# anovos/anovos

Measured on AMD Instinct MI355X. Metric: rows/sec (whole node) full analyzer+drift+transform, higher is better.
Workload: dtype fp32 data + fp64 accumulators; 1 GPU; model=anovos-full-pipeline, rows_per_gpu=125000000, n_cols=201, global_batch=125000000, parallelism=dp1

## Files before the change

anovos_amd/data_analyzer/association_evaluator.py:

```python

from __future__ import annotations

import math
import warnings

import numpy as np
import pandas as pd
import torch

from anovos_amd.core import dist
from anovos_amd.core.dtypes import NULL_CODE
from anovos_amd.data_analyzer.association_eval_varclus import VarClusHi
from anovos_amd.data_analyzer.stats_generator import uniqueCount_computation
from anovos_amd.data_transformer.transformers import (
    attribute_binning,
    cat_to_num_unsupervised,
    imputation_MMM,
    monotonic_binning,
    _event_indicator,
)
from anovos_amd.ops import corr as corr_ops
from anovos_amd.ops import rank as rank_ops
from anovos_amd.shared.utils import attributeType_segregation, normalize_columns
from anovos_amd.shared.tracing import traced
# ... 89 lines not shown
    )
    hit = idf.aux_cache.get(key)
    if hit is not None:
        return hit
    from anovos_amd.ops import backend as _backend
    from anovos_amd.ops.groupby import align_dictionaries

    align_dictionaries(idf, list(cols) + [label_col])

    use_fused = (
        bool(encoding_configs)
        and encoding_configs.get("monotonicity_check", 0) == 0
        and len(num_cols) > 0
        and idf.device.type == "cuda"
        and all(idf.col(c).data.is_cuda for c in cols)
        and _backend.use_hip(idf.col(num_cols[0]).data)
        and all(
            len(idf.col(c).dictionary or []) + 1 <= 8192
            for c in cols
            if idf.col(c).kind == "categorical"
        )
    )
    if use_fused:
        from anovos_amd.data_transformer.transformers import compute_bin_cutoffs

        bin_size = int(encoding_configs["bin_size"])
        bin_method = encoding_configs["bin_method"]
        kept, cutlists = compute_bin_cutoffs(ctx, idf, num_cols, bin_method, bin_size)
        cutmap = dict(zip(kept, cutlists))
        numset = set(num_cols)
        ncols_order = [c for c in cols if c in numset]
        ccols_order = [c for c in cols if c not in numset]
        ext = _backend.hip_ext()
        lab_u8 = label.to(torch.uint8).contiguous()
        nsizes = [bin_size + 2] * len(ncols_order)
        tensors = [idf.col(c).data.contiguous() for c in ncols_order]
        cuts = [torch.tensor(cutmap.get(c, []), dtype=torch.float64) for c in ncols_order]
        parts = [ext.bucketize_label_counts(tensors, cuts, lab_u8, nsizes)]
        csizes = []
        if ccols_order:
            ctensors = []
            for c in ccols_order:
                t = idf.col(c).data
                ctensors.append(t.contiguous() if t.dtype == torch.int32 else t.to(torch.int32).contiguous())
            csizes = [len(idf.col(c).dictionary or []) + 1 for c in ccols_order]
            parts.append(ext.label_counts_multi(ctensors, lab_u8, csizes))
        flat = torch.cat(parts) if len(parts) > 1 else parts[0]
        flat = dist.all_reduce_(flat.to(torch.float64), "sum").cpu().numpy()
        out, off = {}, 0
        for c, s in zip(ncols_order + ccols_order, nsizes + csizes):
            tot = flat[off : off + s]
            n1 = flat[off + s : off + 2 * s]
            out[c] = (tot - n1, n1)
            off += 2 * s
        idf.aux_cache[key] = out
        return out
    nmax = None
    if len(num_cols) > 0 and bool(encoding_configs):
        bin_size = encoding_configs["bin_size"]
        bin_method = encoding_configs["bin_method"]
        if encoding_configs.get("monotonicity_check", 0) == 1:
# ... 391 lines not shown
```

anovos_amd/data_transformer/transformers.py:

```python

from __future__ import annotations

import math
import os
import warnings
from typing import Dict, Optional

import numpy as np
import pandas as pd
import torch

from anovos_amd.core import dist
from anovos_amd.core.dtypes import NULL_CODE
from anovos_amd.core.frame import AnovosFrame, Column
from anovos_amd.ops import bucketize as bucketize_ops
from anovos_amd.ops import encode as encode_ops
from anovos_amd.ops import groupby as groupby_ops
from anovos_amd.ops import histogram as hist_ops
from anovos_amd.ops import stats as stats_ops
from anovos_amd.shared.utils import attributeType_segregation, normalize_columns
from anovos_amd.shared.tracing import traced


def _save_model(pdf: pd.DataFrame, model_path: str, name: str, fmt: str = "parquet"):
# ... 39 lines not shown


@traced
def compute_bin_cutoffs(ctx, idf, list_of_cols, method_type, bin_size):
    if method_type == "equal_frequency":
        pctile_width = 1 / bin_size
        probs = [j * pctile_width for j in range(1, bin_size)]
        q = hist_ops.approx_quantiles(idf, list_of_cols, probs, rel_err=0.01)
        return list_of_cols, [q[c] for c in list_of_cols]
    moments = stats_ops.frame_moments(idf, list_of_cols)
    bin_cutoffs = []
    dropped = []
    for c in list_of_cols:
        m = moments[c]
        if m.max != m.max:
            dropped.append(c)
            continue
        w = (m.max - m.min) / bin_size
        bin_cutoffs.append([m.min + j * w for j in range(1, bin_size)])
    if dropped:
        warnings.warn("Columns contains too much null values. Dropping " + ", ".join(dropped))
        list_of_cols = [c for c in list_of_cols if c not in dropped]
    return list_of_cols, bin_cutoffs


def attribute_binning(
    ctx,
    idf,
    list_of_cols="all",
    drop_cols=[],
    method_type="equal_range",
    bin_size=10,
    bin_dtype="numerical",
    pre_existing_model=False,
    model_path="NA",
    output_mode="replace",
    print_impact=False,
):
    num_cols = attributeType_segregation(idf)[0]
    if list_of_cols == "all":
        list_of_cols = num_cols
    list_of_cols = normalize_columns(idf, list_of_cols, drop_cols, restrict_to=num_cols)
    if any(x not in num_cols for x in list_of_cols):
        raise TypeError("Invalid input for Column(s)")
    if len(list_of_cols) == 0:
        warnings.warn("No Binning Performed - No numerical column(s) to transform")
# ... 848 lines not shown
```

anovos_amd/ops/hip/anovos_bindings.hip:

```cpp

#include <torch/extension.h>
#include <c10/hip/HIPStream.h>
#include <hip/hip_runtime.h>

#include <algorithm>
#include <cstdlib>
#include <cstring>
#include <optional>
#include <vector>

#include "anovos_kernels.h"

namespace {

hipStream_t current_stream() { return c10::hip::getCurrentHIPStream().stream(); }

void check_hip(int err, const char *what) {
  TORCH_CHECK(err == 0, what, " failed: ", hipGetErrorString((hipError_t)err));
}

int pick_chunks(int64_t n, int ncols) {
  int64_t by_size = (n + (1 << 16) - 1) >> 16;
  int64_t cap = std::max<int64_t>(1, 16384 / std::max(1, ncols));
  int64_t c = std::min<int64_t>(std::max<int64_t>(by_size, 1), cap);
// ... 893 lines not shown
  for (int i = 0; i < b.ncols(); ++i) {
    TORCH_CHECK(sizes[i] >= 1 && sizes[i] <= LABEL_MAX_SLOTS, b.name, ": slot count out of LDS range");
    offs.push_back(off);
    off += 2 * sizes[i];
    kinds.push_back(b.dtypes[i] == 2 ? 1 : 0);
    max_slots = std::max(max_slots, (int)sizes[i]);
  }
  int nchunks = pick_chunks(b.maxn, b.ncols());
  auto out = torch::zeros({off}, on(b.device, torch::kInt64));
  auto dptr = upload(b.ptrs, b.device);
  auto dlen = upload(b.lens, b.device);
  auto doff = upload(offs, b.device);
  auto dsz = upload(std::vector<int>(sizes.begin(), sizes.end()), b.device);
  auto dkind = upload(kinds, b.device);
  check_hip(anovos_label_counts_multi(ptr_table<const void>(dptr), label.data_ptr<uint8_t>(),
                                      dlen.data_ptr<int64_t>(), doff.data_ptr<int64_t>(),
                                      dsz.data_ptr<int>(), dkind.data_ptr<int>(), b.ncols(),
                                      max_slots, nchunks, (uint64_t *)out.data_ptr<int64_t>(),
                                      current_stream()),
            "anovos_label_counts_multi");
  return out;
}

torch::Tensor bucketize_label_counts(std::vector<torch::Tensor> cols,
                                     std::vector<torch::Tensor> cutoffs, torch::Tensor label,
                                     std::vector<int64_t> sizes) {
  ColumnBatch all = gather_columns(cols, "bucketize_label_counts", F32 | F64, true);
  check_count(cutoffs.size(), cols.size(), all.name, "cutoffs");
  check_count(sizes.size(), cols.size(), all.name, "sizes");
  check_dense_on_device(label, all, "label", torch::kUInt8, all.maxn);
  auto device = all.device;
  std::vector<int64_t> out_offs;
  int64_t total = 0;
  for (int64_t s : sizes) {
    TORCH_CHECK(s >= 1 && s <= LABEL_MAX_SLOTS, all.name, ": slot count out of LDS range");
    out_offs.push_back(total);
    total += 2 * s;
  }
  auto out = torch::zeros({total}, on(device, torch::kInt64));
  for (auto &b : split_by_dtype(all)) {
    CutoffTable ct = cutoff_table(cutoffs, b.idx);
    auto sz = pick(sizes, b.idx);
    int max_slots = (int)std::max<int64_t>(1, *std::max_element(sz.begin(), sz.end()));
    int nchunks = pick_chunks(b.maxn, b.ncols());
    auto dptr = upload(b.ptrs, device);
    auto dlen = upload(b.lens, device);
    auto doff = upload(pick(out_offs, b.idx), device);
    auto dcoff = upload(ct.offs, device);
    auto dflat = upload(ct.flat, device);
    auto dclen = upload(ct.lens, device);
    auto dsz = upload(std::vector<int>(sz.begin(), sz.end()), device);
    check_hip(anovos_bucketize_label_counts(
                  ptr_table<const void>(dptr), label.data_ptr<uint8_t>(), dlen.data_ptr<int64_t>(),
                  dflat.data_ptr<double>(), dcoff.data_ptr<int64_t>(), dclen.data_ptr<int>(),
                  doff.data_ptr<int64_t>(), dsz.data_ptr<int>(), b.ncols(), ct.max_ncut, max_slots,
                  nchunks, b.dtype, (uint64_t *)out.data_ptr<int64_t>(), current_stream()),
              "anovos_bucketize_label_counts");
  }
  return out;
}

std::tuple<torch::Tensor, std::vector<torch::Tensor>> outlier_clamp_columns(
    std::vector<torch::Tensor> cols, torch::Tensor lo, torch::Tensor hi, int64_t mode) {
  ColumnBatch all = gather_columns(cols, "outlier_clamp_columns", F32 | F64);
  auto device = all.device;
  auto lo_d = device_f64(lo, cols.size(), all, "lo");
  auto hi_d = device_f64(hi, cols.size(), all, "hi");
  auto counts = torch::zeros({all.ncols(), 2}, on(device, torch::kInt64));
  std::vector<torch::Tensor> outs;
  if (mode)
    for (auto &t : cols) outs.push_back(torch::empty_like(t));
  for (auto &b : split_by_dtype(all)) {
    int nchunks = pick_chunks(b.maxn, b.ncols());
    auto dptr = upload(b.ptrs, device);
    auto dlen = upload(b.lens, device);
    auto didx = upload(b.idx, device);
    auto lo_sel = lo_d.index_select(0, didx);
    auto hi_sel = hi_d.index_select(0, didx);
    auto sub = torch::zeros({b.ncols(), 2}, on(device, torch::kInt64));
    torch::Tensor dout;
    if (mode) dout = upload(out_ptrs(outs, b), device);
    check_hip(anovos_outlier_clamp(ptr_table<const void>(dptr), dlen.data_ptr<int64_t>(),
// ... 98 lines not shown
              "anovos_grade_apply");
  }
  return outs;
}

PYBIND11_MODULE(TORCH_EXTENSION_NAME, m) {
  m.def("grade_counts", &grade_counts, "rows per grid cell of each column, read-only (K24)");
  m.def("grade_apply", &grade_apply, "per-cell grade lookup to f32 columns (K24)",
        py::arg("cols"), py::arg("cutoffs"), py::arg("tables"), py::arg("null_grade"),
        py::arg("outs") = py::none());
  m.attr("GRADE_MAX_CELLS") = GRADE_MAX_CELLS;
  m.def("code_counts_multi",&code_counts_multi, "fused multi-column code counts + null slot (K5)",
        py::arg("cols"), py::arg("sizes"), py::arg("null_masks") = false);
  m.def("pair_code_counts", &pair_code_counts, "contingency tables of code-column pairs (K22)");
  m.def("pair_code_counts_plan", &pair_code_counts_plan,
        "[items, column streams, LDS counters] of a K22 pair list");
  m.def("grouped_moments", &grouped_moments, "(n, s1, s2) of value columns per code slot (K23)");
  m.def("grouped_moments_plan", &grouped_moments_plan,
        "[items, column streams, accumulator cells] of a K23 pair list");
  m.attr("GRP_CELLS") = GRP_CELLS;
  m.def("outlier_clamp_columns", &outlier_clamp_columns, "fused outlier count/clamp (K10/K11)");
  m.def("label_counts_multi", &label_counts_multi, "fused multi-column label-conditioned histograms (K9)");
  m.def("bucketize_label_counts", &bucketize_label_counts, "fused bucketize + label counts, no binned materialization (K6+K9)");
  m.def("moments_hll", &moments_hll, "fused moments + HLL registers (K1/K2+K4)",
        py::arg("cols"), py::arg("p"), py::arg("shifts") = std::vector<double>(),
        py::arg("null_masks") = false);
  m.def("centered_gram_bf16", &centered_gram_bf16, "bf16 MFMA centered Gram X^T X (K8)");
  m.def("bracket_histograms_grouped", &bracket_histograms_grouped, "grouped refinement histograms (K3)");
  m.def("bucketize_columns_float", &bucketize_columns_float, "bucketize to float bin labels (K6)");
  m.def("bucketize_columns_float_counts", &bucketize_columns_float_counts,
        "bucketize to float bin labels + per-column bin counts from the same pass (K6)");
  m.def("lut_apply_f32", &lut_apply_f32, "fused LUT gather -> float (K12)");
  m.def("lut_apply_i32", &lut_apply_i32, "fused LUT gather -> int32 (K12)");
  m.def("hll_registers_multi", &hll_registers_multi, "fused multi-column HLL (K4)");
  m.def("scale_columns", &scale_columns, "fused (x-a)*b scaling (K11)");
  m.def("fill_nan_columns", &fill_nan_columns, "fused NaN fill (K11)");
  m.def("fill_code_columns", &fill_code_columns, "fused categorical null fill (K11)");
  m.def("column_moments", &column_moments, "fused per-column moments (K1/K2)",
        py::arg("cols"), py::arg("shifts") = std::vector<double>());
  m.def("column_histograms", &column_histograms, "fused per-column histograms (K3/K6)");
  m.def("bracket_histograms", &bracket_histograms, "quantile-refinement histograms (K3)");
  m.def("bucketize_columns", &bucketize_columns, "branchless bucketize (K6)");
  m.def("code_counts", &code_counts, "dictionary code bincount (K5)");
  m.def("hll_registers", &hll_registers, "HyperLogLog registers (K4)");
  m.def("row_null_counts_num", &row_null_counts_num, "fused row null counts (K10)");
  m.def("row_null_counts_masked", &row_null_counts_masked,
// ... 3 lines not shown
```

anovos_amd/ops/hip/anovos_kernels.h:

```cpp

#pragma once

#include <hip/hip_runtime.h>
#include <cstdint>


constexpr int CODE_LDS_SLOTS = 16384;
constexpr int PAIR_LDS_SLOTS = 16384;
constexpr int PAIR_PMAX = 8;
constexpr int PAIR_ITEM_WORDS = 4 + 4 * PAIR_PMAX;
constexpr int GRP_CELLS = 16;
constexpr int GRP_PMAX = 8;
constexpr int GRP_THREADS = 256;
constexpr int GRP_CELL_BYTES = 20;
constexpr int GRP_ITEM_WORDS = 5 + 2 * GRP_PMAX;
constexpr int RB_BINS = 512;
constexpr int RB_MAXB = 16;
constexpr int LABEL_MAX_SLOTS = 8192;
constexpr int BKT_COUNTS_MAX_NCUT = 4096;
constexpr int GRADE_MAX_CELLS = 4096;
__host__ __device__ constexpr int64_t null_mask_chunk_words(int64_t per) {
  return 4 * ((((per >> 2) + 63) >> 6) + 1);
}


extern "C" {
int anovos_moments(const void *const *cols, const int64_t *lens,
                   const double *shifts, int ncols, int nchunks, int dtype,
                   double *partials, double *out, hipStream_t stream);
int anovos_hist(const void *const *cols, const int64_t *lens, int ncols,
                const double *lo, const double *hi, int nbins, int nchunks,
                int dtype, uint64_t *out, hipStream_t stream);
int anovos_bracket_hist(const void *const *cols, const int64_t *lens,
                        const int64_t *colidx, int nbrackets, const double *lo,
                        const double *hi, int nbins, int nchunks, int dtype,
                        uint64_t *out, hipStream_t stream);
int anovos_bucketize(const void *const *cols, const int64_t *lens, int ncols,
                     const double *cutflat, const int64_t *cutoff_off,
                     const int *cutoff_len, int max_ncut, int nchunks, int dtype,
                     int32_t *const *outs, hipStream_t stream);
int anovos_code_counts(const int32_t *codes, int64_t n, int size, int nchunks,
                       uint64_t *out, hipStream_t stream);
int anovos_hll(const void *x, int64_t n, int p, int nchunks, int dtype,
// ... 38 lines not shown
                             uint64_t *const *masks, hipStream_t stream);
int anovos_outlier_clamp(const void *const *cols, const int64_t *lens,
                         int ncols, const double *lo, const double *hi,
                         int nchunks, int mode, int dtype, void *const *outs,
                         uint64_t *counts, hipStream_t stream);
int anovos_moments_hll(const void *const *cols, const int64_t *lens,
                       const double *shifts, int ncols, int p, int nchunks,
                       int dtype, double *partials, double *mom_out,
                       int32_t *regs, uint64_t *const *masks, hipStream_t stream);
int anovos_row_null_masked(const uint64_t *const *masks, int ncols, int64_t n,
                           int nchunks, int64_t per, int32_t *out,
                           hipStream_t stream);
int anovos_bucketize_label_counts(const void *const *cols, const uint8_t *label,
                                  const int64_t *lens, const double *cutflat,
                                  const int64_t *cutoff_off, const int *cutoff_len,
                                  const int64_t *offs, const int *sizes, int ncols,
                                  int max_ncut, int max_slots, int nchunks,
                                  int dtype, uint64_t *out, hipStream_t stream);
int anovos_label_counts_multi(const void *const *cols, const uint8_t *label,
                              const int64_t *lens, const int64_t *offs,
                              const int *sizes, const int *dtypes, int ncols,
                              int max_slots, int nchunks, uint64_t *out,
                              hipStream_t stream);
int anovos_centered_gram(const void *const *cols, int64_t n, int k,
                         const float *means, const int *pair_i,
                         const int *pair_j, int npairs, int row_chunks,
                         float *partials, float *gram, hipStream_t stream);
int anovos_centered_gram_sr(const void *const *cols, int64_t n, int k,
                            const float *means, const int *pair_i,
                            const int *pair_j, int npairs, int row_chunks,
                            float *partials, float *gram, hipStream_t stream);
int anovos_gram_sr_grid(int k);
int anovos_pair_code_counts(const int32_t *const *cols, const int64_t *items,
                            int nitems, int64_t n, int64_t per, int nchunks,
                            int lds_slots, uint64_t *out, hipStream_t stream);
int anovos_grouped_moments(const int32_t *const *codes, const void *const *vals,
                           const double *shifts, const int64_t *items, int nitems,
                           int64_t n, int64_t per, int nchunks, int cells, int dtype,
                           double *partials, double *out, hipStream_t stream);
int anovos_grade_counts(const void *const *cols, const int64_t *lens, int ncols,
                        const double *cutflat, const int64_t *cutoff_off,
                        const int *cutoff_len, int max_ncut, int nchunks, int dtype,
                        uint64_t *counts, const int64_t *count_off, hipStream_t stream);
int anovos_grade_apply(const void *const *cols, const int64_t *lens, int ncols,
                       const double *cutflat, const int64_t *cutoff_off,
                       const int *cutoff_len, const float *tabflat, const int64_t *tab_off,
// ... 4 lines not shown
```

anovos_amd/ops/hip/anovos_kernels.hip:

```cpp

#include <hip/hip_runtime.h>
#include <cfloat>
#include <cstdint>
#include <cmath>

#include "anovos_kernels.h"

#define THREADS 256
#define DEV_INLINE __device__ __forceinline__

typedef int nat_i4 __attribute__((ext_vector_type(4)));
typedef float nat_f4 __attribute__((ext_vector_type(4)));

#define GLOBAL_AS __attribute__((address_space(1)))
typedef const nat_f4 GLOBAL_AS *gin_f4;
typedef const nat_i4 GLOBAL_AS *gin_i4;

DEV_INLINE int block_column(int nchunks) { return blockIdx.x % (gridDim.x / nchunks); }
DEV_INLINE int block_chunk(int nchunks) { return blockIdx.x / (gridDim.x / nchunks); }

DEV_INLINE int64_t chunk_rows(int64_t n, int nchunks) {
  const uint64_t t = (uint64_t)n + (uint64_t)(nchunks - 1);
  if (t <= 0xFFFFFFFFull) return (int64_t)((uint32_t)t / (uint32_t)nchunks);
  return (int64_t)(t / (uint64_t)nchunks);
// ... 1862 lines not shown
    lds += (size_t)THREADS * 17 * sizeof(uint32_t);
#define BKT_LABEL_F32(NREG)                                                     \
  hipLaunchKernelGGL((bucketize_label_counts_kernel<float, NREG>),              \
                     dim3(ncols * nchunks), dim3(THREADS), lds, stream,         \
                     (const float *const *)cols, label, lens, cutflat,          \
                     cutoff_off, cutoff_len, offs, sizes, max_ncut, max_slots,  \
                     nchunks, out)
  const int nreg = bkt_nreg(max_ncut);
  if (dtype == 0 && nreg == 9)
    BKT_LABEL_F32(9);
  else if (dtype == 0 && nreg == 16)
    BKT_LABEL_F32(16);
  else if (dtype == 0)
    BKT_LABEL_F32(0);
  else
    hipLaunchKernelGGL((bucketize_label_counts_kernel<double, 0>),
                       dim3(ncols * nchunks), dim3(THREADS), lds, stream,
                       (const double *const *)cols, label, lens, cutflat,
                       cutoff_off, cutoff_len, offs, sizes, max_ncut, max_slots,
                       nchunks, out);
#undef BKT_LABEL_F32
  return (int)hipGetLastError();
}
```

anovos_amd/ops/histogram.py:

```python

from __future__ import annotations

from typing import Dict, List, Optional, Sequence

import torch

from anovos_amd.core import dist
from anovos_amd.ops import backend

DEFAULT_BINS = 2048
EXACT_N_THRESHOLD = 250_000
MAX_REFINE_PASSES = 8
_MIN_SPLIT_ULPS = 4 * 2048


def _splittable(bracket):
    import numpy as np

    bl, bh = bracket[0], bracket[1]
    return bh - bl > _MIN_SPLIT_ULPS * float(np.spacing(max(abs(bl), abs(bh))))


def _bracket_extrema(tensors, brackets):
    inf = float("inf")
    uniq = {}
    for k, v in brackets.items():
        uniq.setdefault((k[0], v[0], v[1]), len(uniq))
    dev = tensors[0].device
    red = torch.empty(3, len(uniq), dtype=torch.float64, device=dev)
    red[0], red[1], red[2] = inf, -inf, 0.0
    x64, x64_col = None, None
    for (i, bl, bh), u in sorted(uniq.items()):
        if tensors[i].numel() == 0:
            continue
        if x64_col != i:
            x64, x64_col = tensors[i].to(torch.float64), i
# ... 28 lines not shown
        n = xs.numel()
        if n == 0:
            out[c] = [float("nan")] * len(probs)
            continue
        vals = []
        for p in probs:
            if p <= rel_err:
                r = 1
            elif p >= 1 - rel_err:
                r = n
            else:
                r = min(max(int(_math.ceil(p * n)), 1), n)
            vals.append(float(xs[r - 1]))
        out[c] = vals
    return out


def _exact_integral_quantiles(idf, cols, probs, moments, rel_err=0.0):
    import math as _math

    import numpy as np

    R = {c: int(moments[c].max - moments[c].min) + 1 for c in cols}
    cold = [c for c in cols if ("inthist",) not in idf.col(c).cache]
    if cold:
        M = max(R[c] for c in cold)
        lo = torch.tensor([moments[c].min - 0.5 for c in cold], dtype=torch.float64)
        hi = torch.tensor([moments[c].min - 0.5 + M for c in cold], dtype=torch.float64)
        h = global_histograms([idf.col(c).data for c in cold], lo, hi, M).cpu().numpy()
        for i, c in enumerate(cold):
            idf.col(c).cache[("inthist",)] = (h[i][: R[c]].copy(), float(moments[c].min))
    out = {}
    for c in cols:
        n = int(moments[c].n)
        counts, cmin = idf.col(c).cache[("inthist",)]
        cdf = np.cumsum(counts)
        vals = []
        for p in probs:
            if p <= rel_err:
                r = 1
            elif p >= 1 - rel_err:
                r = n
            else:
                r = min(max(int(_math.ceil(p * n)), 1), n)
            b = int(np.searchsorted(cdf, r, side="left"))
            vals.append(float(cmin + min(b, R[c] - 1)))
        out[c] = vals
    return out


def column_histograms(
    tensors: Sequence[torch.Tensor],
    lo: torch.Tensor,
    hi: torch.Tensor,
# ... 52 lines not shown
        if rest:
            out.update(approx_quantiles(idf, rest, probs_l, nbins=nbins, refine=refine,
                                        moments=moments, rel_err=rel_err))
        return {c: out[c] for c in cols}
    int_cols = [
        c for c in cols
        if moments[c].n > 0 and moments[c].integral
        and moments[c].min == moments[c].min
        and 0 < (moments[c].max - moments[c].min) < 4096
        and any(("q", p) not in idf.col(c).cache for p in probs_l)
    ]
    if int_cols:
        dense = _exact_integral_quantiles(idf, int_cols, probs_l, moments, rel_err=rel_err)
        for c in int_cols:
            for j, p in enumerate(probs_l):
                idf.col(c).cache[("q", p)] = dense[c][j]
        rest = [c for c in cols if c not in set(int_cols)]
        if not rest:
            return {c: [idf.col(c).cache[("q", p)] for p in probs_l] for c in cols}
        out = approx_quantiles(idf, rest, probs_l, nbins=nbins, refine=refine,
                               moments=moments, rel_err=rel_err)
        out.update(dense)
        return {c: out[c] for c in cols}
    lo = torch.tensor([moments[c].min for c in cols], dtype=torch.float64)
    hi = torch.tensor([moments[c].max for c in cols], dtype=torch.float64)
    probs = list(probs)

    key = ("hist", nbins)
    todo = [i for i, c in enumerate(cols) if key not in idf.col(c).cache]
    if todo:
        tensors = [idf.col(cols[i]).data for i in todo]
        h = global_histograms(tensors, lo[todo], hi[todo], nbins).cpu()
        for k, i in enumerate(todo):
            idf.col(cols[i]).cache[key] = h[k]
    import numpy as np

    hist_np = torch.stack([idf.col(c).cache[key] for c in cols]).numpy().astype(np.float64)
    cdf = np.cumsum(hist_np, axis=1)
    tensors = [idf.col(c).data for c in cols]

    result = {c: [float("nan")] * len(probs) for c in cols}
    brackets = {}
    top = set()
    probs_np = np.asarray(probs)
    K, P = len(cols), len(probs)
    ns = np.array([moments[c].n for c in cols], dtype=np.float64)
    lows = lo.numpy().astype(np.float64)
    highs = hi.numpy().astype(np.float64)
    valid = (ns > 0) & (lows == lows)
    degenerate = valid & (highs <= lows)
    for i in np.nonzero(degenerate)[0]:
        result[cols[i]] = [float(lows[i])] * P
    active = np.nonzero(valid & ~degenerate)[0]
    if active.size:
        w = (highs[active] - lows[active]) / nbins
        targets = probs_np[None, :] * (ns[active, None] - 1)
        cdf_a = cdf[active]
        bs = np.minimum((cdf_a[:, :, None] < (targets + 0.5)[:, None, :]).sum(axis=1), nbins - 1)
        rows = np.arange(active.size)[:, None]
        belows = np.where(bs > 0, cdf_a[rows, np.maximum(bs - 1, 0)], 0.0)
        cnts = hist_np[active][rows, bs]
        for a, i in enumerate(active):
            l = lows[i]
            wa = w[a]
            for j in range(P):
                b = int(bs[a, j])
                brackets[(int(i), j)] = (l + b * wa, l + (b + 1) * wa, float(targets[a, j] - belows[a, j]), float(cnts[a, j]))
        top = {(int(active[a]), int(j)) for a, j in zip(*np.nonzero(bs == nbins - 1))}
    thr = {int(i): rel_err * 0.5 * max(ns[i], 1.0) for i in active}
    point = {}
    unresolved = set()
    passes = MAX_REFINE_PASSES if refine is None else refine
    over = True
    for it in range(passes):
        need = {
            k: v for k, v in brackets.items()
            if v[3] > thr[k[0]] and k not in point and k[0] not in unresolved
        }
        over = bool(need)
        need = {k: v for k, v in need.items() if _splittable(v)}
        if not need:
            break
        if it == 0:
            for k in need:
                if k in top:
                    need[k] = (need[k][0], float(np.nextafter(highs[k[0]], np.inf))) + need[k][2:]
        refined = _refine_pass(tensors, cols, need, nbins, lo, hi)
        stuck = {}
        for k, v in refined.items():
            if v[4] != need[k][3]:
                unresolved.add(k[0])
            elif v[3] == need[k][3]:
                stuck[k] = need[k]
            brackets[k] = v[:4]
        stuck = {k: v for k, v in stuck.items() if k[0] not in unresolved}
        if stuck:
            for k, (mn, mx) in _bracket_extrema(tensors, stuck).items():
                if not mn <= mx:
                    unresolved.add(k[0])
                elif mn == mx:
                    point[k] = mn
                else:
                    brackets[k] = (mn, float(np.nextafter(mx, np.inf))) + stuck[k][2:]
    left = {
        k: v for k, v in brackets.items()
        if v[3] > 2.0 * thr[k[0]] and k not in point and k[0] not in unresolved
    } if over else {}
    if left:
        for k, (mn, mx) in _bracket_extrema(tensors, left).items():
            if mn == mx:
                point[k] = mn
            else:
                unresolved.add(k[0])
    for (i, j), (bl, bh, off, cnt) in brackets.items():
        c = cols[i]
        if cnt <= 1 or bh <= bl:
            result[c][j] = bl
        else:
            frac = min(max(off / max(cnt - 1, 1e-9), 0.0), 1.0) if cnt > 1 else 0.0
            result[c][j] = bl + frac * (bh - bl)
    for (i, j), v in point.items():
        result[cols[i]][j] = v
    for i, j in top:
        result[cols[i]][j] = min(result[cols[i]][j], float(highs[i]))
    if unresolved:
        result.update(_exact_quantiles(idf, [cols[i] for i in sorted(unresolved)], probs, moments, rel_err=rel_err))
    for c in cols:
        for j, p in enumerate(probs_l):
            idf.col(c).cache[("q", p)] = result[c][j]
    return result


def _refine_pass(tensors, cols, brackets, nbins, col_lo=None, col_hi=None):
    if not brackets:
        return brackets
    all_keys = sorted(brackets.keys())
    uniq = {}
    key_to_uniq = {}
    for k in all_keys:
        u = (k[0], brackets[k][0], brackets[k][1])
        if u not in uniq:
            uniq[u] = len(uniq)
        key_to_uniq[k] = uniq[u]
    keys = [None] * len(uniq)
    for k in all_keys:
        if keys[key_to_uniq[k]] is None:
            keys[key_to_uniq[k]] = k
    dev = tensors[0].device
    blo = torch.tensor([brackets[k][0] for k in keys], dtype=torch.float64)
    bhi = torch.tensor([brackets[k][1] for k in keys], dtype=torch.float64)
    colidx = torch.tensor([k[0] for k in keys], dtype=torch.int64)
    if dev.type == "cuda" and backend.use_hip(tensors[0]):
        ext = backend.hip_ext()
# ... 82 lines not shown
```

Before: 489.2 million rows/sec.

## Compute equal-frequency bin cutoffs on device and feed bucketize kernel directly

Adds HIP kernels that compute quantiles from device-resident histograms and dense integer counts, and a bucketize_label_counts variant that takes cutoffs as a device matrix. In the IV/IG fused path, equal-frequency cutoffs are computed on the GPU when the cached histograms allow it. This skips host round-trips, the numpy bracket search and re-uploading the cutoffs. Columns whose histogram bins are too coarse still fall back to the host refinement path. The cost is more code paths and cache-dependent conditions that decide which path runs.

```diff
diff --git a/anovos_amd/data_analyzer/association_evaluator.py b/anovos_amd/data_analyzer/association_evaluator.py
--- a/anovos_amd/data_analyzer/association_evaluator.py
+++ b/anovos_amd/data_analyzer/association_evaluator.py
@@ -135,12 +135,10 @@
         )
     )
     if use_fused:
-        from anovos_amd.data_transformer.transformers import compute_bin_cutoffs
+        from anovos_amd.data_transformer.transformers import _device_bin_cutoffs, compute_bin_cutoffs
 
         bin_size = int(encoding_configs["bin_size"])
         bin_method = encoding_configs["bin_method"]
-        kept, cutlists = compute_bin_cutoffs(ctx, idf, num_cols, bin_method, bin_size)
-        cutmap = dict(zip(kept, cutlists))
         numset = set(num_cols)
         ncols_order = [c for c in cols if c in numset]
         ccols_order = [c for c in cols if c not in numset]
@@ -148,8 +146,14 @@
         lab_u8 = label.to(torch.uint8).contiguous()
         nsizes = [bin_size + 2] * len(ncols_order)
         tensors = [idf.col(c).data.contiguous() for c in ncols_order]
-        cuts = [torch.tensor(cutmap.get(c, []), dtype=torch.float64) for c in ncols_order]
-        parts = [ext.bucketize_label_counts(tensors, cuts, lab_u8, nsizes)]
+        cut_matrix = _device_bin_cutoffs(idf, ncols_order, bin_method, bin_size)
+        if cut_matrix is not None:
+            parts = [ext.bucketize_label_counts_dev(tensors, cut_matrix, lab_u8, nsizes)]
+        else:
+            kept, cutlists = compute_bin_cutoffs(ctx, idf, num_cols, bin_method, bin_size)
+            cutmap = dict(zip(kept, cutlists))
+            cuts = [torch.tensor(cutmap.get(c, []), dtype=torch.float64) for c in ncols_order]
+            parts = [ext.bucketize_label_counts(tensors, cuts, lab_u8, nsizes)]
         csizes = []
         if ccols_order:
             ctensors = []
diff --git a/anovos_amd/data_transformer/transformers.py b/anovos_amd/data_transformer/transformers.py
--- a/anovos_amd/data_transformer/transformers.py
+++ b/anovos_amd/data_transformer/transformers.py
@@ -85,6 +85,14 @@
         warnings.warn("Columns contains too much null values. Dropping " + ", ".join(dropped))
         list_of_cols = [c for c in list_of_cols if c not in dropped]
     return list_of_cols, bin_cutoffs
+
+
+def _device_bin_cutoffs(idf, list_of_cols, method_type, bin_size):
+    if method_type != "equal_frequency":
+        return None
+    pctile_width = 1 / bin_size
+    probs = [j * pctile_width for j in range(1, bin_size)]
+    return hist_ops.device_quantile_matrix(idf, list_of_cols, probs, rel_err=0.01)
 
 
 def attribute_binning(
diff --git a/anovos_amd/ops/hip/anovos_bindings.hip b/anovos_amd/ops/hip/anovos_bindings.hip
--- a/anovos_amd/ops/hip/anovos_bindings.hip
+++ b/anovos_amd/ops/hip/anovos_bindings.hip
@@ -939,11 +939,25 @@
   return out;
 }
 
-torch::Tensor bucketize_label_counts(std::vector<torch::Tensor> cols,
-                                     std::vector<torch::Tensor> cutoffs, torch::Tensor label,
-                                     std::vector<int64_t> sizes) {
-  ColumnBatch all = gather_columns(cols, "bucketize_label_counts", F32 | F64, true);
-  check_count(cutoffs.size(), cols.size(), all.name, "cutoffs");
+namespace {
+torch::Tensor bucketize_label_counts_body(const std::vector<torch::Tensor> &cols,
+                                          const std::vector<torch::Tensor> *cutoffs,
+                                          const torch::Tensor *cut_matrix,
+                                          const torch::Tensor &label,
+                                          const std::vector<int64_t> &sizes, const char *name) {
+  ColumnBatch all = gather_columns(cols, name, F32 | F64, true);
+  int64_t ncut = 0;
+  if (cutoffs) {
+    check_count(cutoffs->size(), cols.size(), all.name, "cutoffs");
+  } else {
+    TORCH_CHECK(cut_matrix->dim() == 2 && cut_matrix->size(0) == (int64_t)cols.size() &&
+                    cut_matrix->size(1) >= 1 && cut_matrix->size(1) <= LABEL_MAX_SLOTS,
+                all.name, ": cut_matrix must be [ncols, ncut] with 1 <= ncut <= ", LABEL_MAX_SLOTS);
+    TORCH_CHECK(cut_matrix->device() == all.device && cut_matrix->is_contiguous() &&
+                    cut_matrix->scalar_type() == torch::kFloat64,
+                all.name, ": cut_matrix must be a contiguous float64 tensor on the columns' device");
+    ncut = cut_matrix->size(1);
+  }
   check_count(sizes.size(), cols.size(), all.name, "sizes");
   check_dense_on_device(label, all, "label", torch::kUInt8, all.maxn);
   auto device = all.device;
@@ -956,7 +970,17 @@
   }
   auto out = torch::zeros({total}, on(device, torch::kInt64));
   for (auto &b : split_by_dtype(all)) {
-    CutoffTable ct = cutoff_table(cutoffs, b.idx);
+    CutoffTable ct;
+    torch::Tensor dflat;
+    if (cutoffs) {
+      ct = cutoff_table(*cutoffs, b.idx);
+      dflat = upload(ct.flat, device);
+    } else {
+      for (int64_t i : b.idx) ct.offs.push_back(i * ncut);
+      ct.lens.assign(b.idx.size(), (int)ncut);
+      ct.max_ncut = (int)ncut;
+      dflat = *cut_matrix;
+    }
     auto sz = pick(sizes, b.idx);
     int max_slots = (int)std::max<int64_t>(1, *std::max_element(sz.begin(), sz.end()));
     int nchunks = pick_chunks(b.maxn, b.ncols());
@@ -964,7 +988,6 @@
     auto dlen = upload(b.lens, device);
     auto doff = upload(pick(out_offs, b.idx), device);
     auto dcoff = upload(ct.offs, device);
-    auto dflat = upload(ct.flat, device);
     auto dclen = upload(ct.lens, device);
     auto dsz = upload(std::vector<int>(sz.begin(), sz.end()), device);
     check_hip(anovos_bucketize_label_counts(
@@ -975,6 +998,79 @@
               "anovos_bucketize_label_counts");
   }
   return out;
+}
+
+const double *query_param(const torch::Tensor &t, int64_t ncols, const torch::Device &dev,
+                          const char *name, const char *what) {
+  TORCH_CHECK(t.device() == dev && t.is_contiguous() && t.scalar_type() == torch::kFloat64 &&
+                  t.numel() == ncols,
+              name, ": ", what, " must be a contiguous float64 tensor of ", ncols,
+              " entries on the histogram's device");
+  return t.data_ptr<double>();
+}
+
+void check_query_matrix(const torch::Tensor &h, const std::vector<double> &probs, const char *name) {
+  TORCH_CHECK(h.is_cuda() && h.dim() == 2 && h.is_contiguous() && h.scalar_type() == torch::kInt64,
+              name, ": expected a contiguous int64 [ncols, nbins] device tensor");
+  TORCH_CHECK(h.size(0) >= 1 && h.size(1) >= 1 && h.size(1) <= QQ_MAX_BINS, name,
+              ": need at least one column and 1 .. ", QQ_MAX_BINS, " bins");
+  TORCH_CHECK(!probs.empty(), name, ": no probabilities");
+}
+}
+
+torch::Tensor bucketize_label_counts(std::vector<torch::Tensor> cols,
+                                     std::vector<torch::Tensor> cutoffs, torch::Tensor label,
+                                     std::vector<int64_t> sizes) {
+  return bucketize_label_counts_body(cols, &cutoffs, nullptr, label, sizes,
+                                     "bucketize_label_counts");
+}
+
+torch::Tensor bucketize_label_counts_dev(std::vector<torch::Tensor> cols, torch::Tensor cut_matrix,
+                                         torch::Tensor label, std::vector<int64_t> sizes) {
+  return bucketize_label_counts_body(cols, nullptr, &cut_matrix, label, sizes,
+                                     "bucketize_label_counts_dev");
+}
+
+std::tuple<torch::Tensor, torch::Tensor, torch::Tensor> hist_quantile_query(
+    torch::Tensor hist, torch::Tensor lo, torch::Tensor hi, torch::Tensor n,
+    std::vector<double> probs, double rel_err) {
+  const char *name = "hist_quantile_query";
+  check_query_matrix(hist, probs, name);
+  const int64_t ncols = hist.size(0), P = (int64_t)probs.size();
+  auto dev = hist.device();
+  const double *plo = query_param(lo, ncols, dev, name, "lo");
+  const double *phi = query_param(hi, ncols, dev, name, "hi");
+  const double *pn = query_param(n, ncols, dev, name, "n");
+  auto vals = torch::empty({ncols, P}, on(dev, torch::kFloat64));
+  auto flags = torch::empty({ncols, P}, on(dev, torch::kUInt8));
+  auto maxbin = torch::empty({ncols}, on(dev, torch::kInt64));
+  auto dprobs = upload(probs, dev);
+  check_hip(anovos_hist_quantile_query((const uint64_t *)hist.data_ptr<int64_t>(), plo, phi, pn,
+                                       dprobs.data_ptr<double>(), rel_err, (int)ncols,
+                                       (int)hist.size(1), (int)P, vals.data_ptr<double>(),
+                                       flags.data_ptr<uint8_t>(), maxbin.data_ptr<int64_t>(),
+                                       current_stream()),
+            "anovos_hist_quantile_query");
+  return {vals, flags, maxbin};
+}
+
+torch::Tensor inthist_quantile_query(torch::Tensor counts, torch::Tensor cmin, torch::Tensor n,
+                                     torch::Tensor R, std::vector<double> probs, double rel_err) {
+  const char *name = "inthist_quantile_query";
+  check_query_matrix(counts, probs, name);
+  const int64_t ncols = counts.size(0), P = (int64_t)probs.size();
+  auto dev = counts.device();
+  const double *pmin = query_param(cmin, ncols, dev, name, "cmin");
+  const double *pn = query_param(n, ncols, dev, name, "n");
+  const double *pR = query_param(R, ncols, dev, name, "R");
+  auto vals = torch::empty({ncols, P}, on(dev, torch::kFloat64));
+  auto dprobs = upload(probs, dev);
+  check_hip(anovos_inthist_quantile_query((const uint64_t *)counts.data_ptr<int64_t>(),
+                                          (int)counts.size(1), pmin, pn, pR,
+                                          dprobs.data_ptr<double>(), rel_err, (int)ncols, (int)P,
+                                          vals.data_ptr<double>(), current_stream()),
+            "anovos_inthist_quantile_query");
+  return vals;
 }
 
 std::tuple<torch::Tensor, std::vector<torch::Tensor>> outlier_clamp_columns(
@@ -1119,6 +1215,11 @@
   m.def("outlier_clamp_columns", &outlier_clamp_columns, "fused outlier count/clamp (K10/K11)");
   m.def("label_counts_multi", &label_counts_multi, "fused multi-column label-conditioned histograms (K9)");
   m.def("bucketize_label_counts", &bucketize_label_counts, "fused bucketize + label counts, no binned materialization (K6+K9)");
+  m.def("bucketize_label_counts_dev", &bucketize_label_counts_dev,
+        "bucketize_label_counts with the cutoffs as a device [ncols, ncut] matrix (K6+K9)");
+  m.def("hist_quantile_query", &hist_quantile_query, "quantiles of device-resident histograms (K3q)");
+  m.def("inthist_quantile_query", &inthist_quantile_query,
+        "exact quantiles of device-resident dense integer counts (K3q)");
   m.def("moments_hll", &moments_hll, "fused moments + HLL registers (K1/K2+K4)",
         py::arg("cols"), py::arg("p"), py::arg("shifts") = std::vector<double>(),
         py::arg("null_masks") = false);
diff --git a/anovos_amd/ops/hip/anovos_kernels.h b/anovos_amd/ops/hip/anovos_kernels.h
--- a/anovos_amd/ops/hip/anovos_kernels.h
+++ b/anovos_amd/ops/hip/anovos_kernels.h
@@ -19,6 +19,7 @@
 constexpr int LABEL_MAX_SLOTS = 8192;
 constexpr int BKT_COUNTS_MAX_NCUT = 4096;
 constexpr int GRADE_MAX_CELLS = 4096;
+constexpr int QQ_MAX_BINS = 4096;
 __host__ __device__ constexpr int64_t null_mask_chunk_words(int64_t per) {
   return 4 * ((((per >> 2) + 63) >> 6) + 1);
 }
@@ -103,6 +104,14 @@
                               const int *sizes, const int *dtypes, int ncols,
                               int max_slots, int nchunks, uint64_t *out,
                               hipStream_t stream);
+int anovos_hist_quantile_query(const uint64_t *hist, const double *lo, const double *hi,
+                               const double *n, const double *probs, double rel_err,
+                               int ncols, int nbins, int P, double *vals, uint8_t *flags,
+                               int64_t *maxbin, hipStream_t stream);
+int anovos_inthist_quantile_query(const uint64_t *counts, int rows, const double *cmin,
+                                  const double *n, const double *R, const double *probs,
+                                  double rel_err, int ncols, int P, double *vals,
+                                  hipStream_t stream);
 int anovos_centered_gram(const void *const *cols, int64_t n, int k,
                          const float *means, const int *pair_i,
                          const int *pair_j, int npairs, int row_chunks,
diff --git a/anovos_amd/ops/hip/anovos_kernels.hip b/anovos_amd/ops/hip/anovos_kernels.hip
--- a/anovos_amd/ops/hip/anovos_kernels.hip
+++ b/anovos_amd/ops/hip/anovos_kernels.hip
@@ -1908,3 +1908,141 @@
 #undef BKT_LABEL_F32
   return (int)hipGetLastError();
 }
+
+
+DEV_INLINE uint64_t qq_prefix(const uint64_t *__restrict__ h, int nb, uint64_t *cdf,
+                              uint64_t *part, uint64_t *pmax) {
+  const int per = (nb + THREADS - 1) / THREADS;
+  const int s = min(nb, (int)threadIdx.x * per);
+  const int e = min(nb, s + per);
+  uint64_t run = 0, mx = 0;
+  for (int i = s; i < e; ++i) {
+    const uint64_t c = h[i];
+    run += c;
+    mx = c > mx ? c : mx;
+    cdf[i] = run;
+  }
+  part[threadIdx.x] = run;
+  pmax[threadIdx.x] = mx;
+  __syncthreads();
+  uint64_t before = 0, allmax = 0;
+  for (int t = 0; t < THREADS; ++t) {
+    before += t < (int)threadIdx.x ? part[t] : 0;
+    allmax = pmax[t] > allmax ? pmax[t] : allmax;
+  }
+  for (int i = s; i < e; ++i) cdf[i] += before;
+  __syncthreads();
+  return allmax;
+}
+
+DEV_INLINE int qq_count_below(const uint64_t *cdf, int nb, double t) {
+  int lo = 0, len = nb;
+  while (len > 0) {
+    const int half = len >> 1;
+    const bool lt = (double)cdf[lo + half] < t;
+    lo = lt ? lo + half + 1 : lo;
+    len = lt ? len - half - 1 : half;
+  }
+  return lo;
+}
+
+__global__ __launch_bounds__(THREADS) void hist_quantile_query_kernel(
+    const uint64_t *__restrict__ hist, const double *__restrict__ lo,
+    const double *__restrict__ hi, const double *__restrict__ n,
+    const double *__restrict__ probs, double rel_err, int nbins, int P,
+    double *__restrict__ vals, uint8_t *__restrict__ flags, int64_t *__restrict__ maxbin) {
+#pragma clang fp contract(off)
+  __shared__ uint64_t cdf[QQ_MAX_BINS];
+  __shared__ uint64_t part[THREADS];
+  __shared__ uint64_t pmax[THREADS];
+  const int col = blockIdx.x;
+  const uint64_t mx = qq_prefix(hist + (size_t)col * nbins, nbins, cdf, part, pmax);
+  if (threadIdx.x == 0) maxbin[col] = (int64_t)mx;
+  const double l = lo[col], h = hi[col], nn = n[col];
+  for (int j = threadIdx.x; j < P; j += THREADS) {
+    double v;
+    bool over = false;
+    if (!(nn > 0.0) || l != l) {
+      v = __longlong_as_double(0x7ff8000000000000LL);
+    } else if (h <= l) {
+      v = l;
+    } else {
+      const double target = probs[j] * (nn - 1.0);
+      const int a = qq_count_below(cdf, nbins, target + 0.5);
+      const int b = a < nbins - 1 ? a : nbins - 1;
+      const uint64_t cb = b > 0 ? cdf[b - 1] : 0;
+      const double below = (double)cb;
+      const double cnt = (double)(cdf[b] - cb);
+      const double w = (h - l) / (double)nbins;
+      const double bl = l + (double)b * w;
+      const double bh = l + (double)(b + 1) * w;
+      if (cnt <= 1.0 || bh <= bl) {
+        v = bl;
+      } else {
+        const double den = cnt - 1.0;
+        double frac = (target - below) / (1e-9 > den ? 1e-9 : den);
+        frac = 0.0 > frac ? 0.0 : frac;
+        frac = 1.0 < frac ? 1.0 : frac;
+        v = bl + frac * (bh - bl);
+      }
+      if (b == nbins - 1) v = h < v ? h : v;
+      const double nmax = 1.0 > nn ? 1.0 : nn;
+      over = cnt > rel_err * 0.5 * nmax;
+    }
+    vals[(size_t)col * P + j] = v;
+    flags[(size_t)col * P + j] = over ? 1 : 0;
+  }
+}
+
+__global__ __launch_bounds__(THREADS) void inthist_quantile_query_kernel(
+    const uint64_t *__restrict__ counts, int rows, const double *__restrict__ cmin,
+    const double *__restrict__ n, const double *__restrict__ Rf,
+    const double *__restrict__ probs, double rel_err, int P, double *__restrict__ vals) {
+#pragma clang fp contract(off)
+  __shared__ uint64_t cdf[QQ_MAX_BINS];
+  __shared__ uint64_t part[THREADS];
+  __shared__ uint64_t pmax[THREADS];
+  const int col = blockIdx.x;
+  int R = (int)Rf[col];
+  R = R < 1 ? 1 : (R > rows ? rows : R);
+  qq_prefix(counts + (size_t)col * rows, R, cdf, part, pmax);
+  const double nn = n[col], c0 = cmin[col];
+  for (int j = threadIdx.x; j < P; j += THREADS) {
+    const double p = probs[j];
+    double r;
+    if (p <= rel_err) {
+      r = 1.0;
+    } else if (p >= 1.0 - rel_err) {
+      r = nn;
+    } else {
+      r = ceil(p * nn);
+      r = 1.0 > r ? 1.0 : r;
+      r = nn < r ? nn : r;
+    }
+    const int a = qq_count_below(cdf, R, r);
+    const int b = a < R - 1 ? a : R - 1;
+    vals[(size_t)col * P + j] = c0 + (double)b;
+  }
+}
+
+extern "C" int anovos_hist_quantile_query(const uint64_t *hist, const double *lo,
+                                          const double *hi, const double *n,
+                                          const double *probs, double rel_err, int ncols,
+                                          int nbins, int P, double *vals, uint8_t *flags,
+                                          int64_t *maxbin, hipStream_t stream) {
+  if (nbins < 1 || nbins > QQ_MAX_BINS || P < 1 || ncols < 1) return (int)hipErrorInvalidValue;
+  hipLaunchKernelGGL(hist_quantile_query_kernel, dim3(ncols), dim3(THREADS), 0, stream, hist,
+                     lo, hi, n, probs, rel_err, nbins, P, vals, flags, maxbin);
+  return (int)hipGetLastError();
+}
+
+extern "C" int anovos_inthist_quantile_query(const uint64_t *counts, int rows,
+                                             const double *cmin, const double *n,
+                                             const double *R, const double *probs,
+                                             double rel_err, int ncols, int P, double *vals,
+                                             hipStream_t stream) {
+  if (rows < 1 || rows > QQ_MAX_BINS || P < 1 || ncols < 1) return (int)hipErrorInvalidValue;
+  hipLaunchKernelGGL(inthist_quantile_query_kernel, dim3(ncols), dim3(THREADS), 0, stream,
+                     counts, rows, cmin, n, R, probs, rel_err, P, vals);
+  return (int)hipGetLastError();
+}
diff --git a/anovos_amd/ops/histogram.py b/anovos_amd/ops/histogram.py
--- a/anovos_amd/ops/histogram.py
+++ b/anovos_amd/ops/histogram.py
@@ -1,6 +1,7 @@
 
 from __future__ import annotations
 
+import os
 from typing import Dict, List, Optional, Sequence
 
 import torch
@@ -12,6 +13,83 @@
 EXACT_N_THRESHOLD = 250_000
 MAX_REFINE_PASSES = 8
 _MIN_SPLIT_ULPS = 4 * 2048
+QQ_MAX_BINS = 4096
+
+
+def device_quantiles_enabled() -> bool:
+    return os.environ.get("ANOVOS_DEVICE_QUANTILES", "1") != "0"
+
+
+def _on_hip(idf, cols) -> bool:
+    t = idf.col(cols[0]).data
+    return t.device.type == "cuda" and backend.use_hip(t)
+
+
+def _pass1_brackets(hist_np, lows, highs, ns, probs):
+    import numpy as np
+
+    nbins = hist_np.shape[1]
+    cdf = np.cumsum(hist_np, axis=1)
+    brackets = {}
+    top = set()
+    probs_np = np.asarray(probs)
+    P = len(probs)
+    lows = np.asarray(lows).astype(np.float64)
+    valid = (ns > 0) & (lows == lows)
+    degenerate = valid & (highs <= lows)
+    constant = {int(i): float(lows[i]) for i in np.nonzero(degenerate)[0]}
+    active = np.nonzero(valid & ~degenerate)[0]
+    if active.size:
+        w = (highs[active] - lows[active]) / nbins
+        targets = probs_np[None, :] * (ns[active, None] - 1)
+        cdf_a = cdf[active]
+        bs = np.minimum((cdf_a[:, :, None] < (targets + 0.5)[:, None, :]).sum(axis=1), nbins - 1)
+        rows = np.arange(active.size)[:, None]
+        belows = np.where(bs > 0, cdf_a[rows, np.maximum(bs - 1, 0)], 0.0)
+        cnts = hist_np[active][rows, bs]
+        for a, i in enumerate(active):
+            l = lows[i]
+            wa = w[a]
+            for j in range(P):
+                b = int(bs[a, j])
+                brackets[(int(i), j)] = (l + b * wa, l + (b + 1) * wa, float(targets[a, j] - belows[a, j]), float(cnts[a, j]))
+        top = {(int(active[a]), int(j)) for a, j in zip(*np.nonzero(bs == nbins - 1))}
+    return constant, active, brackets, top
+
+
+def _bracket_values(brackets, point, top, highs):
+    out = {}
+    for k, (bl, bh, off, cnt) in brackets.items():
+        if cnt <= 1 or bh <= bl:
+            out[k] = bl
+        else:
+            frac = min(max(off / max(cnt - 1, 1e-9), 0.0), 1.0) if cnt > 1 else 0.0
+            out[k] = bl + frac * (bh - bl)
+    for k, v in point.items():
+        out[k] = v
+    for k in top:
+        out[k] = min(out[k], float(highs[k[0]]))
+    return out
+
+
+def host_quantile_query(hist, lo, hi, n, probs, rel_err):
+    import numpy as np
+
+    hist_np = np.asarray(hist).astype(np.float64)
+    lows = np.asarray(lo, dtype=np.float64)
+    highs = np.asarray(hi, dtype=np.float64)
+    ns = np.asarray(n, dtype=np.float64)
+    K, P = hist_np.shape[0], len(probs)
+    vals = np.full((K, P), float("nan"))
+    flags = np.zeros((K, P), dtype=bool)
+    constant, active, brackets, top = _pass1_brackets(hist_np, lows, highs, ns, list(probs))
+    for i, v in constant.items():
+        vals[i, :] = v
+    for (i, j), v in _bracket_values(brackets, {}, top, highs).items():
+        vals[i, j] = v
+    for (i, j), v in brackets.items():
+        flags[i, j] = v[3] > rel_err * 0.5 * max(ns[i], 1.0)
+    return vals, flags, hist_np.max(axis=1)
 
 
 def _splittable(bracket):
@@ -86,14 +164,26 @@
     import numpy as np
 
     R = {c: int(moments[c].max - moments[c].min) + 1 for c in cols}
-    cold = [c for c in cols if ("inthist",) not in idf.col(c).cache]
+    use_dev = device_quantiles_enabled() and _on_hip(idf, cols)
+    dkey = ("inthist_dev",)
+    cold = [c for c in cols if ("inthist",) not in idf.col(c).cache or (use_dev and dkey not in idf.col(c).cache)]
     if cold:
         M = max(R[c] for c in cold)
         lo = torch.tensor([moments[c].min - 0.5 for c in cold], dtype=torch.float64)
         hi = torch.tensor([moments[c].min - 0.5 + M for c in cold], dtype=torch.float64)
-        h = global_histograms([idf.col(c).data for c in cold], lo, hi, M).cpu().numpy()
+        hd = global_histograms([idf.col(c).data for c in cold], lo, hi, M)
+        if use_dev:
+            meta = torch.tensor([[moments[c].min for c in cold], [float(int(moments[c].n)) for c in cold],
+                                 [float(R[c]) for c in cold]], dtype=torch.float64).to(hd.device)
+            for i, c in enumerate(cold):
+                idf.col(c).cache[dkey] = (hd, meta, i)
+    vals_d = _device_integral_query(idf, cols, probs, rel_err) if use_dev else None
+    if cold:
+        h = hd.cpu().numpy()
         for i, c in enumerate(cold):
             idf.col(c).cache[("inthist",)] = (h[i][: R[c]].copy(), float(moments[c].min))
+    if vals_d is not None:
+        return dict(zip(cols, vals_d.cpu().tolist()))
     out = {}
     for c in cols:
         n = int(moments[c].n)
@@ -192,12 +282,121 @@
                                moments=moments, rel_err=rel_err)
         out.update(dense)
         return {c: out[c] for c in cols}
+    if device_quantiles_enabled() and nbins <= QQ_MAX_BINS and _on_hip(idf, cols):
+        H, meta = _device_histograms(idf, cols, nbins, moments)
+        dv, df, dm = backend.hip_ext().hist_quantile_query(H, meta[0], meta[1], meta[2], probs_l, float(rel_err))
+        vals, flagged, maxbin = dv.cpu().tolist(), df.cpu().numpy().any(axis=1), dm.cpu().tolist()
+        host_cols = []
+        for i, c in enumerate(cols):
+            idf.col(c).cache[("hist_maxbin", nbins)] = maxbin[i]
+            if flagged[i]:
+                host_cols.append(c)
+            else:
+                for j, p in enumerate(probs_l):
+                    idf.col(c).cache[("q", p)] = vals[i][j]
+        out = _host_bracket_quantiles(idf, cols, probs_l, nbins, refine, moments, rel_err, only=host_cols) if host_cols else {}
+        return {c: out[c] if c in out else vals[i] for i, c in enumerate(cols)}
+    return _host_bracket_quantiles(idf, cols, probs_l, nbins, refine, moments, rel_err)
+
+
+def _device_histograms(idf, cols, nbins, moments):
+    dkey = ("hist_dev", nbins)
+    todo = [c for c in cols if dkey not in idf.col(c).cache]
+    if todo:
+        lo = torch.tensor([moments[c].min for c in todo], dtype=torch.float64)
+        hi = torch.tensor([moments[c].max for c in todo], dtype=torch.float64)
+        h = global_histograms([idf.col(c).data for c in todo], lo, hi, nbins)
+        n = torch.tensor([moments[c].n for c in todo], dtype=torch.float64)
+        meta = torch.stack([lo, hi, n]).to(h.device)
+        for k, c in enumerate(todo):
+            idf.col(c).cache[dkey] = (h, meta, k)
+    return _gather_cached_rows([idf.col(c).cache[dkey] for c in cols])
+
+
+def _gather_cached_rows(entries):
+    base, meta, _ = entries[0]
+    if all(e[0] is base for e in entries) and [e[2] for e in entries] == list(range(base.shape[0])):
+        return base, meta
+    if any(e[0].shape[1] != base.shape[1] for e in entries):
+        return None, None
+    return (torch.stack([e[0][e[2]] for e in entries]),
+            torch.stack([e[1][:, e[2]] for e in entries], dim=1).contiguous())
+
+
+def _device_integral_query(idf, cols, probs, rel_err):
+    counts, meta = _gather_cached_rows([idf.col(c).cache[("inthist_dev",)] for c in cols])
+    if counts is None:
+        return None
+    return backend.hip_ext().inthist_quantile_query(counts, meta[0], meta[1], meta[2], list(probs), float(rel_err))
+
+
+def _is_dense_integral(m) -> bool:
+    return bool(m.n > 0 and m.integral and m.min == m.min and 0 < (m.max - m.min) < 4096)
+
+
+def device_quantile_matrix(idf, cols, probs, nbins: int = DEFAULT_BINS, rel_err: float = 1e-2):
+    import math as _math
+
+    from anovos_amd.ops import stats as stats_ops
+
+    probs = list(probs)
+    if not cols or not probs or not device_quantiles_enabled() or nbins > QQ_MAX_BINS or not _on_hip(idf, cols):
+        return None
+    moments = stats_ops.frame_moments(idf, cols)
+    if all(moments[c].n <= EXACT_N_THRESHOLD for c in cols):
+        return None
+    if all(all(("q", p) in idf.col(c).cache for p in probs) for c in cols):
+        held = [[idf.col(c).cache[("q", p)] for p in probs] for c in cols]
+        return torch.tensor(held, dtype=torch.float64).to(idf.col(cols[0]).data.device)
+    hist_cols, int_cols = [], []
+    for c in cols:
+        m, cache = moments[c], idf.col(c).cache
+        if _math.isinf(m.min) or _math.isinf(m.max):
+            return None
+        if _is_dense_integral(m):
+            if ("inthist_dev",) not in cache or all(("q", p) in cache for p in probs):
+                return None
+            int_cols.append(c)
+        else:
+            mb = cache.get(("hist_maxbin", nbins))
+            if mb is None or ("hist_dev", nbins) not in cache:
+                return None
+            ranged = m.n > 0 and m.min == m.min and not m.max <= m.min
+            if ranged and mb > rel_err * 0.5 * max(m.n, 1.0):
+                return None
+            hist_cols.append(c)
+    ext = backend.hip_ext()
+    parts = []
+    if hist_cols:
+        H, meta = _device_histograms(idf, hist_cols, nbins, moments)
+        parts.append(ext.hist_quantile_query(H, meta[0], meta[1], meta[2], probs, float(rel_err))[0])
+    if int_cols:
+        v = _device_integral_query(idf, int_cols, probs, rel_err)
+        if v is None:
+            return None
+        parts.append(v)
+    out = torch.cat(parts) if len(parts) > 1 else parts[0]
+    order = hist_cols + int_cols
+    if order != list(cols):
+        pos = {c: i for i, c in enumerate(order)}
+        out = out.index_select(0, torch.tensor([pos[c] for c in cols], dtype=torch.long).to(out.device))
+    return out.contiguous()
+
+
+def _host_bracket_quantiles(idf, cols, probs, nbins, refine, moments, rel_err, only=None):
+    probs_l = probs
+    picked = list(cols) if only is None else [c for c in cols if c in set(only)]
     lo = torch.tensor([moments[c].min for c in cols], dtype=torch.float64)
     hi = torch.tensor([moments[c].max for c in cols], dtype=torch.float64)
-    probs = list(probs)
 
     key = ("hist", nbins)
-    todo = [i for i, c in enumerate(cols) if key not in idf.col(c).cache]
+    for c in picked:
+        cache = idf.col(c).cache
+        if key not in cache and ("hist_dev", nbins) in cache:
+            h, _, row = cache[("hist_dev", nbins)]
+            cache[key] = h[row].cpu()
+    pos = {c: i for i, c in enumerate(cols)}
+    todo = [pos[c] for c in picked if key not in idf.col(c).cache]
     if todo:
         tensors = [idf.col(cols[i]).data for i in todo]
         h = global_histograms(tensors, lo[todo], hi[todo], nbins).cpu()
@@ -205,38 +404,17 @@
             idf.col(cols[i]).cache[key] = h[k]
     import numpy as np
 
-    hist_np = torch.stack([idf.col(c).cache[key] for c in cols]).numpy().astype(np.float64)
-    cdf = np.cumsum(hist_np, axis=1)
+    skip = set(cols) - set(picked)
+    empty = torch.zeros(nbins, dtype=torch.int64)
+    hist_np = torch.stack([empty if c in skip else idf.col(c).cache[key] for c in cols]).numpy().astype(np.float64)
     tensors = [idf.col(c).data for c in cols]
 
     result = {c: [float("nan")] * len(probs) for c in cols}
-    brackets = {}
-    top = set()
-    probs_np = np.asarray(probs)
-    K, P = len(cols), len(probs)
-    ns = np.array([moments[c].n for c in cols], dtype=np.float64)
-    lows = lo.numpy().astype(np.float64)
+    ns = np.array([0.0 if c in skip else moments[c].n for c in cols], dtype=np.float64)
     highs = hi.numpy().astype(np.float64)
-    valid = (ns > 0) & (lows == lows)
-    degenerate = valid & (highs <= lows)
-    for i in np.nonzero(degenerate)[0]:
-        result[cols[i]] = [float(lows[i])] * P
-    active = np.nonzero(valid & ~degenerate)[0]
-    if active.size:
-        w = (highs[active] - lows[active]) / nbins
-        targets = probs_np[None, :] * (ns[active, None] - 1)
-        cdf_a = cdf[active]
-        bs = np.minimum((cdf_a[:, :, None] < (targets + 0.5)[:, None, :]).sum(axis=1), nbins - 1)
-        rows = np.arange(active.size)[:, None]
-        belows = np.where(bs > 0, cdf_a[rows, np.maximum(bs - 1, 0)], 0.0)
-        cnts = hist_np[active][rows, bs]
-        for a, i in enumerate(active):
-            l = lows[i]
-            wa = w[a]
-            for j in range(P):
-                b = int(bs[a, j])
-                brackets[(int(i), j)] = (l + b * wa, l + (b + 1) * wa, float(targets[a, j] - belows[a, j]), float(cnts[a, j]))
-        top = {(int(active[a]), int(j)) for a, j in zip(*np.nonzero(bs == nbins - 1))}
+    constant, active, brackets, top = _pass1_brackets(hist_np, lo.numpy(), highs, ns, probs)
+    for i, v in constant.items():
+        result[cols[i]] = [v] * len(probs)
     thr = {int(i): rel_err * 0.5 * max(ns[i], 1.0) for i in active}
     point = {}
     unresolved = set()
@@ -282,23 +460,14 @@
                 point[k] = mn
             else:
                 unresolved.add(k[0])
-    for (i, j), (bl, bh, off, cnt) in brackets.items():
-        c = cols[i]
-        if cnt <= 1 or bh <= bl:
-            result[c][j] = bl
-        else:
-            frac = min(max(off / max(cnt - 1, 1e-9), 0.0), 1.0) if cnt > 1 else 0.0
-            result[c][j] = bl + frac * (bh - bl)
-    for (i, j), v in point.items():
+    for (i, j), v in _bracket_values(brackets, point, top, highs).items():
         result[cols[i]][j] = v
-    for i, j in top:
-        result[cols[i]][j] = min(result[cols[i]][j], float(highs[i]))
     if unresolved:
         result.update(_exact_quantiles(idf, [cols[i] for i in sorted(unresolved)], probs, moments, rel_err=rel_err))
-    for c in cols:
+    for c in picked:
         for j, p in enumerate(probs_l):
             idf.col(c).cache[("q", p)] = result[c][j]
-    return result
+    return {c: result[c] for c in picked}
 
 
 def _refine_pass(tensors, cols, brackets, nbins, col_lo=None, col_hi=None):
```

Measured after the change: 516.9 million rows/sec (median of 6 runs). 5.7% higher.
